# UZ-SLAMLab/ORB_SLAM3

Hardware: AMD Instinct MI355X
Metric: ORB kfeatures/sec extract+match, EuRoC 752x480 nFeatures=1000 (higher is better)
Workload: dtype u8

## Files before the change

include/orbx.h:

```cpp
#ifndef ORBX_H
#define ORBX_H

#include <stddef.h>
#include <stdint.h>

#ifdef __cplusplus
extern "C" {
#endif

#define ORBX_VERSION 100

enum {
    ORBX_OK = 0,
    ORBX_E_EMPTY = -1,
    ORBX_E_BAD_ARG = -2,
    ORBX_E_TOO_SMALL = -3,
    ORBX_E_CAPACITY = -4,
    ORBX_E_NO_DEVICE = -5,
    ORBX_E_HIP = -6,
    ORBX_E_TOO_LARGE = -7,
    ORBX_E_INTERNAL = -8,
    ORBX_E_STALE = -9
};

// ... 52 lines not shown
int orbx_batch_download(orbx_extractor *ex, int frame, orbx_keypoint *keypoints, uint8_t *descriptors, int cap,
                        int *n_out, int *mono_index);
int orbx_batch_download_all(orbx_extractor *ex, orbx_keypoint *keypoints, uint8_t *descriptors, int32_t *counts,
                            int32_t *mono_index);
int orbx_output_capacity(orbx_extractor *ex, int width, int height);
int orbx_batch_download_async(orbx_extractor *ex, orbx_keypoint *keypoints, uint8_t *descriptors, int32_t *counts,
                              int32_t *mono_index, int32_t *match, int32_t *nmatches);
int orbx_download_wait(orbx_extractor *ex);

int orbx_get_level(orbx_extractor *ex, int frame, int level, uint8_t *dst, size_t dst_stride);
int orbx_level_size(orbx_extractor *ex, int width, int height, int level, int *w, int *h);
int orbx_get_level_device(orbx_extractor *ex, int frame, int level, const uint8_t **d_padded, size_t *pitch);

int orbx_get_levels(const orbx_extractor *ex);
float orbx_get_scale_factor(const orbx_extractor *ex);
int orbx_get_scale_tables(const orbx_extractor *ex, float *scale, float *inv_scale, float *sigma2, float *inv_sigma2);
int orbx_get_feature_tables(const orbx_extractor *ex, int32_t *features_per_level, int32_t *umax16);

int orbx_debug_level_candidates(orbx_extractor *ex, int frame, int level, orbx_keypoint *out, int cap);
int orbx_debug_level_keypoints(orbx_extractor *ex, int frame, int level, orbx_keypoint *out, int cap);
int orbx_debug_level_blurred(orbx_extractor *ex, int frame, int level, uint8_t *dst, size_t dst_stride);
int orbx_debug_fused_patches(orbx_extractor *ex, int frame, uint8_t *dst, int cap_keypoints);
int orbx_debug_stage_stats(orbx_extractor *ex, int64_t *out, int cap);

int orbx_tune_fast_queues(orbx_extractor *ex, int mode, int32_t info[4]);

int orbx_profile_enable(orbx_extractor *ex, int enable);
int orbx_profile_read(orbx_extractor *ex, const char **names, double *avg_ms, int64_t *launches, int cap);

typedef struct orbx_matcher orbx_matcher;
int orbx_matcher_create(int device, orbx_matcher **out);
void orbx_matcher_destroy(orbx_matcher *m);
int orbx_matcher_debug_transfers(const orbx_matcher *m, int64_t *out, int cap);
int orbx_matcher_debug_replay_stats(const orbx_matcher *m, int32_t *out3);

#define ORBX_TH_LOW 50
#define ORBX_TH_HIGH 100
#define ORBX_HISTO_LENGTH 30

int orbx_hamming_csr(orbx_matcher *m, const uint8_t *q_desc, int n_q, const uint8_t *t_desc, int n_t,
                     const int32_t *row_ptr, const int32_t *cand, uint16_t *dist_out);

int orbx_hamming_best2_csr(orbx_matcher *m, const uint8_t *q_desc, int n_q, const uint8_t *t_desc, int n_t,
                           const int32_t *row_ptr, const int32_t *cand, int32_t *best_pos, int32_t *best_dist,
                           int32_t *second_pos, int32_t *second_dist);

// ... 271 lines not shown
```

orb_slam3_amd/_lib.py:

```python
from __future__ import annotations

import ctypes as C
import os
from pathlib import Path

import numpy as np

_PKG = Path(__file__).resolve().parent
LIB_PATH = _PKG / "liborbx.so"

KP_DTYPE = np.dtype([("x", "<f4"), ("y", "<f4"), ("size", "<f4"), ("angle", "<f4"), ("response", "<f4"),
                     ("octave", "<i4"), ("class_id", "<i4")])

ORBX_OK = 0
ORBX_E_EMPTY = -1
ORBX_E_STALE = -9
FLAG_DESC_STRICT = 1
FLAG_BLUR_OCV440 = 2
FLAG_ATAN_FMA = 4
TH_LOW, TH_HIGH, HISTO_LENGTH = 50, 100, 30


class OrbxError(RuntimeError):
    def __init__(self, status: int, where: str):
# ... 73 lines not shown
class BowKeyFrame(C.Structure):
    _fields_ = [("descriptors", C.c_void_p), ("angle", C.c_void_p), ("valid", C.c_void_p), ("n", C.c_int32), ("fv", FeatVec)]


MAX_BOW_KEYFRAMES = 1024


class FuseQueries(C.Structure):
    _fields_ = [("n", C.c_int32), ("u", C.c_void_p), ("v", C.c_void_p), ("ur", C.c_void_p), ("r", C.c_void_p), ("level", C.c_void_p),
                ("desc", C.c_void_p)]


MAX_FUSE_KEYFRAMES = 256

PAIR_PREDICATE = C.CFUNCTYPE(C.c_int, C.c_void_p, C.c_int, C.c_int)

_lib = None

SYMBOLS = [
    "orbx_create", "orbx_destroy", "orbx_extract", "orbx_extract_batch_device", "orbx_extract_batch_host", "orbx_batch_view_get", "orbx_sync",
    "orbx_batch_download", "orbx_batch_download_all", "orbx_batch_download_async", "orbx_download_wait", "orbx_output_capacity", "orbx_get_level", "orbx_level_size",
    "orbx_get_level_device", "orbx_get_levels", "orbx_get_scale_factor", "orbx_get_scale_tables",
    "orbx_get_feature_tables", "orbx_debug_level_candidates", "orbx_debug_level_keypoints",
    "orbx_debug_level_blurred", "orbx_debug_stage_stats", "orbx_tune_fast_queues", "orbx_debug_fused_patches", "orbx_profile_enable", "orbx_profile_read", "orbx_matcher_create",
    "orbx_matcher_destroy", "orbx_matcher_debug_transfers", "orbx_matcher_debug_replay_stats", "orbx_hamming_csr", "orbx_hamming_best2_csr", "orbx_knn2", "orbx_stereo_rowband",
    "orbx_compute_stereo_matches", "orbx_search_by_projection_mappoints", "orbx_search_by_projection_frame",
    "orbx_match_consecutive_device", "orbx_last_error", "orbx_status_string", "orbx_search_by_projection_window", "orbx_search_by_projection_mappoints_fisheye", "orbx_search_by_projection_frame_fisheye",
    "orbx_search_by_bow_frame_fisheye", "orbx_undistort_keypoints", "orbx_image_bounds", "orbx_is_in_frustum", "orbx_is_in_frustum_checks", "orbx_frustum_batch_device",
    "orbx_set_camera", "orbx_batch_download_keypoints_un",
    "orbx_search_for_initialization", "orbx_search_by_bow_frame", "orbx_search_by_bow_keyframes",
    "orbx_search_for_triangulation", "orbx_search_for_triangulation_pinhole", "orbx_search_for_triangulation_kb8", "orbx_debug_kb8_epipolar", "orbx_stereo_batch_device", "orbx_stereo_batch_download", "orbx_stereo_batch_download_all", "orbx_stereo_batch_download_async", "orbx_stereo_download_wait", "orbx_search_mappoints_batch_device", "orbx_vocabulary_create",
    "orbx_vocabulary_destroy", "orbx_bow_transform", "orbx_distinctive_descriptors", "orbx_fuse_search",
    "orbx_frame_create", "orbx_frame_destroy", "orbx_frame_load_host", "orbx_frame_load_batch", "orbx_frame_count",
    "orbx_frame_search_by_projection_mappoints", "orbx_frame_search_by_projection_frame", "orbx_frame_search_local_points",
    "orbx_compute_stereo_fisheye_matches", "orbx_stereo_fisheye_batch_device", "orbx_stereo_fisheye_batch_download",
    "orbx_stereo_fisheye_batch_download_all",
    "orbx_vocabulary_set_word_weights", "orbx_frame_compute_bow", "orbx_frame_search_by_bow", "orbx_frame_search_by_projection_window",
    "orbx_frame_load_host_fisheye", "orbx_frame_load_stereo_fisheye_batch", "orbx_frame_counts", "orbx_frame_search_by_projection_mappoints_fisheye",
    "orbx_frame_search_by_projection_frame_fisheye", "orbx_frame_search_local_points_fisheye",
    "orbx_frame_compute_bow_fisheye", "orbx_frame_search_by_bow_fisheye", "orbx_frame_search_by_projection_window_fisheye",
    "orbx_keyframe_from_frame", "orbx_keyframe_create_host", "orbx_keyframe_count", "orbx_keyframe_destroy", "orbx_keyframe_fuse_search",
    "orbx_keyframe_fuse_map_points",
]


def lib() -> C.CDLL:
    global _lib
# ... 12 lines not shown
    L.orbx_destroy.argtypes = [vp]
    L.orbx_extract.argtypes = [vp, vp, i32, i32, sz, i32, i32, vp, vp, i32, vp, vp]
    L.orbx_extract_batch_device.argtypes = [vp, vp, i32, i32, i32, sz, sz, i32, i32]
    L.orbx_extract_batch_host.argtypes = [vp, vp, i32, i32, i32, sz, sz, i32, i32]
    L.orbx_batch_view_get.argtypes = [vp, C.POINTER(BatchView)]
    L.orbx_sync.argtypes = [vp]
    L.orbx_batch_download.argtypes = [vp, i32, vp, vp, i32, vp, vp]
    L.orbx_batch_download_all.argtypes = [vp, vp, vp, vp, vp]
    L.orbx_output_capacity.argtypes = [vp, i32, i32]
    L.orbx_batch_download_async.argtypes = [vp, vp, vp, vp, vp, vp, vp]
    L.orbx_download_wait.argtypes = [vp]
    L.orbx_get_level.argtypes = [vp, i32, i32, vp, sz]
    L.orbx_level_size.argtypes = [vp, i32, i32, i32, vp, vp]
    L.orbx_get_level_device.argtypes = [vp, i32, i32, vp, vp]
    L.orbx_get_levels.argtypes = [vp]
    L.orbx_get_scale_factor.argtypes = [vp]
    L.orbx_get_scale_factor.restype = f32
    L.orbx_get_scale_tables.argtypes = [vp, vp, vp, vp, vp]
    L.orbx_get_feature_tables.argtypes = [vp, vp, vp]
    L.orbx_debug_level_candidates.argtypes = [vp, i32, i32, vp, i32]
    L.orbx_debug_level_keypoints.argtypes = [vp, i32, i32, vp, i32]
    L.orbx_debug_level_blurred.argtypes = [vp, i32, i32, vp, sz]
    L.orbx_debug_stage_stats.argtypes = [vp, vp, i32]
    L.orbx_tune_fast_queues.argtypes = [vp, i32, vp]
    L.orbx_debug_fused_patches.argtypes = [vp, i32, vp, i32]
    L.orbx_debug_sort_nodes.argtypes = [i32, vp, vp, i32, vp]
    L.orbx_debug_sort_nodes_par.argtypes = [i32, vp, vp, i32, vp, vp]
    L.orbx_profile_enable.argtypes = [vp, i32]
    L.orbx_profile_read.argtypes = [vp, vp, vp, vp, i32]
    L.orbx_matcher_create.argtypes = [i32, C.POINTER(vp)]
    L.orbx_matcher_destroy.argtypes = [vp]
    L.orbx_matcher_debug_transfers.argtypes = [vp, vp, i32]
    L.orbx_matcher_debug_replay_stats.argtypes = [vp, vp]
    L.orbx_hamming_csr.argtypes = [vp, vp, i32, vp, i32, vp, vp, vp]
    L.orbx_hamming_best2_csr.argtypes = [vp, vp, i32, vp, i32, vp, vp, vp, vp, vp, vp]
    L.orbx_knn2.argtypes = [vp, vp, i32, vp, i32, vp, vp]
    L.orbx_stereo_rowband.argtypes = [vp, vp, vp, i32, vp, vp, i32, vp, i32, i32, f32, f32, vp, vp]
    L.orbx_compute_stereo_matches.argtypes = [vp, vp, vp, i32, vp, vp, i32, vp, vp, i32, vp, vp, vp, vp, vp, f32, f32,
                                              vp, vp]
    L.orbx_search_by_projection_mappoints.argtypes = [vp, C.POINTER(FrameDesc), vp, i32, vp, vp, vp, vp, vp, vp, vp,
                                                      vp, f32, f32, vp]
    L.orbx_search_by_projection_frame.argtypes = [vp, C.POINTER(FrameDesc), vp, i32, vp, vp, vp, vp, vp, vp, vp, f32,
                                                  i32, i32, vp]
    L.orbx_search_by_projection_mappoints_fisheye.argtypes = [vp, C.POINTER(FrameDesc), vp, i32, vp, vp, vp, i32] + [vp] * 12 + [f32, f32, vp]
    L.orbx_search_by_projection_frame_fisheye.argtypes = [vp, C.POINTER(FrameDesc), vp, i32, vp, i32] + [vp] * 8 + [f32, i32, i32, vp]
    L.orbx_search_by_bow_frame_fisheye.argtypes = [vp, vp, vp, vp, i32, C.POINTER(FeatVec), vp, vp, i32, i32, C.POINTER(FeatVec), f32, i32, vp]
# ... 79 lines not shown
```

orb_slam3_amd/csrc/extractor_state.h:

```cpp
#pragma once

#include <hip/hip_runtime.h>

#include <cstdio>
#include <cstdlib>
#include <string>
#include <vector>

#include "orbx_internal.h"

namespace orbx {

extern thread_local std::string g_last_error;
void set_error(const std::string &s);

#define ORBX_HIP(expr)                                                                                 \
    do {                                                                                               \
        hipError_t _e = (expr);                                                                        \
        if (_e != hipSuccess) {                                                                        \
            orbx::set_error(std::string(#expr) + ": " + hipGetErrorString(_e));                        \
            return ORBX_E_HIP;                                                                         \
        }                                                                                              \
    } while (0)

// ... 66 lines not shown
    typedef orbx::DevBuf DevBuf;
    typedef orbx::LevelInfo LevelInfo;
    enum { K_COUNT = orbx::K_COUNT };
    orbx_params prm;
    int device = 0;
    hipStream_t stream = nullptr;
    std::vector<float> scale, inv_scale, sigma2, inv_sigma2;
    std::vector<int> quota;
    int umax[16];
    int width = 0, height = 0, batch_cap = 0, last_batch = 0;
    std::vector<LevelInfo> lv;
    size_t pyr_frame = 0, blur_frame = 0, cand_frame = 0, lvl_frame = 0;
    int total_cells = 0, cap = 0, max_pool = 0;
    size_t fast_lds = 0;
    bool resize_march_ok[orbx::kMaxLevels] = {};
    bool fast_strip = false;
    static constexpr int kStripGcap0 = 512, kStripQcap0 = 816;
    int strip_gmax = 1024, strip_qmax = 4096;
    int n_strips = 0, strip_pix_bytes = 0, strip_gcap = kStripGcap0, strip_qcap = kStripQcap0;
    int fast_wave_pitch = 64, fast_wave_rows = 0, fast_wave_qfull = 16;
    DevBuf d_fast_ovf;
    bool oct_par = true;
    bool oct_single_wave = false;
    bool fast_wave = true;
    int n_fast_tiles = 0, n_blur_items = 0;
    int blur_waves = 2048;
    DevBuf d_lv, d_xtab, d_ytab, d_xgtab, d_fast_tiles, d_strips, d_blur_items, d_dc;
    struct PyrPlanDev { DevBuf cols, steps, tasks, band0; orbx::PyrStreamGeom geom; int bands = 0; size_t lds = 0; bool ok = false; };
    PyrPlanDev ps_plan[4];
    bool ps_ok = false;
    int ps_wg_target = 512;
    int ps_min_frames = 48;
    bool lvl0_inplace = false;
    bool in0_released = false;
    unsigned in0_copy_seq = 0;
    hipEvent_t in0_event = nullptr;
    const uint8_t *in0_images = nullptr;
    size_t in0_row_stride = 0, in0_frame_stride = 0;
    int n_strips0 = 0;
    DevBuf d_pyr2;
    bool pyr_double = false;
    int pyr_slot = 0;
    uint8_t *pyr_cur() const { return (uint8_t *)(pyr_slot ? d_pyr2.p : d_pyr.p); }
    DevBuf d_pyr, d_blur, d_cellcnt, d_cellent, d_keys0, d_keys1, d_nof0, d_nof1, d_lvlkp, d_lvlcnt, d_candtot, d_work;
    DevBuf d_kps, d_desc, d_count, d_mono, d_err;
    DevBuf d_mkey1, d_mkey2, d_mocc, d_mentries, d_mprobs, d_mres, d_mscale, d_mgrid;
// ... 70 lines not shown
```

orb_slam3_amd/csrc/octree_par.hip.h:

```cpp
#pragma once

#include "octree.hip.h"

namespace orbx {

constexpr int kOctParLdsKeys = 4096;
constexpr int kOctTier1Keys = 1792;
constexpr int kOctBlkE = 17;

#define OCT_WAVE_SYNC() do { __builtin_amdgcn_fence(__ATOMIC_SEQ_CST, "workgroup"); __builtin_amdgcn_wave_barrier(); } while (0)

__host__ __device__ inline size_t oct_par_pool_bytes(int pool) {
    return ((size_t)kOctStackInts * 4 + (size_t)pool * (16 + 16 + 16 + 8 + 16 + 14) + 160 + 15) & ~(size_t)15;
}
__host__ __device__ inline size_t oct_par_lds_bytes(int pool) { return oct_par_pool_bytes(pool) + (size_t)kOctParLdsKeys * 6; }

struct OctBnd { int16_t x0, y0, x1, y1; };
struct OctSeg { int32_t beg, cnt; };

__device__ __forceinline__ uint64_t oct_readlane64(uint64_t v, int l) {
    return ((uint64_t)(uint32_t)__builtin_amdgcn_readlane((int)(v >> 32), l) << 32) | (uint32_t)__builtin_amdgcn_readlane((int)v, l);
}
__device__ __forceinline__ int oct_median3(uint64_t va, uint64_t vb, uint64_t vc, int ia, int ib, int ic) {
    if (oct_less(va, vb)) {
        if (oct_less(vb, vc)) return ib;
        if (oct_less(va, vc)) return ic;
        return ia;
    }
    if (oct_less(va, vc)) return ia;
    if (oct_less(vb, vc)) return ic;
// ... 160 lines not shown
    const int tid = threadIdx.x, lane = tid & 63, w = tid >> 6;
    int run = 0;
    for (int c0 = 0; c0 < ncell; c0 += 256) {
        const int c = c0 + tid;
        const int n = (c < ncell) ? ccnt[c] : 0;
        const int incl = wave_incl_scan(n);
        if (lane == 63) wsum[w] = incl;
        __syncthreads();
        const int s0 = wsum[0], s1 = wsum[1], s2 = wsum[2], s3 = wsum[3];
        __syncthreads();
        const int excl = run + incl - n + (w > 0 ? s0 : 0) + (w > 1 ? s1 : 0) + (w > 2 ? s2 : 0);
        const uint32_t *src = ent + (size_t)c * L.cell_cap;
        for (int k = 0; k < n; k += 4) {
            uint32_t v[4];
#pragma unroll
            for (int u = 0; u < 4; u++) v[u] = (k + u < n) ? src[k + u] : 0u;
#pragma unroll
            for (int u = 0; u < 4; u++) if (k + u < n) dst[excl + k + u] = v[u];
        }
        run += s0 + s1 + s2 + s3;
    }
    return run;
}
template <int CTRL, int ROWS>
__device__ __forceinline__ void oct_seg_step(uint32_t &lo, uint32_t &hi, int &f) {
    const uint32_t plo = (uint32_t)__builtin_amdgcn_update_dpp(0, (int)lo, CTRL, ROWS, 0xf, false);
    const uint32_t phi = (uint32_t)__builtin_amdgcn_update_dpp(0, (int)hi, CTRL, ROWS, 0xf, false);
    const int pf = __builtin_amdgcn_update_dpp(0, f, CTRL, ROWS, 0xf, false);
    if (!f) { lo += plo; hi += phi; }
    f |= pf;
}
__device__ __forceinline__ uint64_t oct_blk_seg_excl(uint64_t v, bool fl, uint64_t *wtot, int *wflag, int lane, int wave) {
    uint32_t lo = (uint32_t)v, hi = (uint32_t)(v >> 32);
    int f = fl ? 1 : 0;
    oct_seg_step<0x111, 0xf>(lo, hi, f);
    oct_seg_step<0x112, 0xf>(lo, hi, f);
    oct_seg_step<0x114, 0xf>(lo, hi, f);
    oct_seg_step<0x118, 0xf>(lo, hi, f);
    oct_seg_step<0x142, 0xa>(lo, hi, f);
    oct_seg_step<0x143, 0xc>(lo, hi, f);
    if (lane == 63) { wtot[wave] = ((uint64_t)hi << 32) | lo; wflag[wave] = f; }
    __syncthreads();
    const uint32_t elo = (uint32_t)__builtin_amdgcn_update_dpp(0, (int)lo, 0x138, 0xf, 0xf, false);
    const uint32_t ehi = (uint32_t)__builtin_amdgcn_update_dpp(0, (int)hi, 0x138, 0xf, 0xf, false);
    const int ef = __builtin_amdgcn_update_dpp(0, f, 0x138, 0xf, 0xf, false);
    const uint64_t ev = ((uint64_t)ehi << 32) | elo;
// ... 525 lines not shown
    OCT_SYNC_ALL();
    for (int i = tid; i < C; i += NT) {
        const uint32_t key = kb[cur][i];
        atomicMax(&best[nof[cur][i]], ((uint32_t)key_s(key) << 20) | (0xfffffu - (uint32_t)i));
    }
    OCT_SYNC_ALL();
    for (int i = tid; i < nn && i < L.lvl_cap; i += NT) {
        const uint32_t key = kb[cur][0xfffffu - (best[i] & 0xfffffu)];
        out[i] = pack_key(key_x(key) + kBorder, key_y(key) + kBorder, key_s(key));
    }
    if (tid == 0) {
        if (nn > L.lvl_cap) atomicExch(err, 3);
        *lvlcnt_out = min(nn, L.lvl_cap);
    }
    OCT_TICK(6);
    if (dbg && tid == 0) { dbg[0] += (long long)wall_clock64() - tstart; dbg[9] = C; dbg[11] = nn; }
#undef OCT_TICK
#undef OCT_SYNC_ALL
}

__device__ __forceinline__ bool oct_blk_form(const LevelInfo &L, int C) { return C <= kOctParLdsKeys && L.nIni <= 4 && L.pool <= 2047; }

template <int KEYS, int LO>
__global__ __launch_bounds__(256, (KEYS <= 2048 ? 5 : 3)) void k_octree_par_t(const LevelInfo *__restrict__ lv, size_t ent_frame_stride,
                                                                              uint32_t *__restrict__ keys1, uint32_t *__restrict__ lvlkp,
                                                                              size_t lvlkp_frame_stride, int32_t *__restrict__ lvlcnt, int nlevels,
                                                                              int32_t *__restrict__ cand_total, int32_t *__restrict__ err,
                                                                              int max_pool, const int32_t *__restrict__ cellcnt, int total_cells,
                                                                              const uint32_t *__restrict__ cellent) {
    extern __shared__ __attribute__((aligned(16))) uint8_t smem[];
    const int level = blockIdx.y, f = blockIdx.x;
    const LevelInfo L = lv[level];
    uint32_t *gk1 = keys1 + (size_t)f * ent_frame_stride + L.cand_off;
    int C;
    if (LO < 0 && cellcnt) {
        C = __builtin_amdgcn_readfirstlane(compact_level(L, cellcnt + (size_t)f * total_cells + L.cell_base,
                                                         cellent + (size_t)f * ent_frame_stride + L.cand_off, gk1));
        if (threadIdx.x == 0) cand_total[f * nlevels + level] = C;
        __syncthreads();
    } else C = __builtin_amdgcn_readfirstlane(cand_total[f * nlevels + level]);
    if (!(C > LO && C <= KEYS && L.nIni <= 4 && L.pool <= 2047)) return;
    octree_par_body<true, KEYS>(L, smem, max_pool, C, nullptr, gk1, nullptr, nullptr, lvlkp + (size_t)f * lvlkp_frame_stride + L.lvl_off,
                                lvlcnt + f * nlevels + level, err, nullptr);
}

__global__ __launch_bounds__(256, 3) void k_octree_rest(const LevelInfo *__restrict__ lv, size_t ent_frame_stride, uint32_t *__restrict__ keys0,
                                                        uint32_t *__restrict__ keys1, uint16_t *__restrict__ nof0, uint16_t *__restrict__ nof1,
                                                        uint32_t *__restrict__ lvlkp, size_t lvlkp_frame_stride, int32_t *__restrict__ lvlcnt,
                                                        int nlevels, const int32_t *__restrict__ cand_total, int32_t *__restrict__ err, int max_pool, int single_wave) {
    extern __shared__ __attribute__((aligned(16))) uint8_t smem[];
    const int level = blockIdx.y, f = blockIdx.x;
    const LevelInfo L = lv[level];
    int32_t *cnt_out = lvlcnt + f * nlevels + level;
    const int C = __builtin_amdgcn_readfirstlane(cand_total[f * nlevels + level]);
    uint32_t *gk1 = keys1 + (size_t)f * ent_frame_stride + L.cand_off;
    if (oct_blk_form(L, C)) {
        if (C <= kOctTier1Keys) return;
        octree_par_body<true, kOctParLdsKeys>(L, smem, max_pool, C, nullptr, gk1, nullptr, nullptr, lvlkp + (size_t)f * lvlkp_frame_stride + L.lvl_off, cnt_out,
                                              err, nullptr);
        return;
    }
    uint32_t *gk0 = keys0 + (size_t)f * ent_frame_stride + L.cand_off;
// ... 16 lines not shown
```

orb_slam3_amd/csrc/orbx_extractor.hip:

```cpp
#include <hip/hip_runtime.h>

#include <algorithm>
#include <cmath>
#include <cstdio>
#include <cstdlib>
#include <cstring>
#include <dlfcn.h>
#include <mutex>
#include <string>
#include <vector>

#include "extractor_kernels.hip.h"
#include "geometry_kernels.hip.h"
#include "extractor_state.h"

namespace orbx {

thread_local std::string g_last_error;

void set_error(const std::string &s) { g_last_error = s; }

namespace {
struct Roctx {
    int (*push)(const char *) = nullptr;
// ... 526 lines not shown
    ex->n_strips = (int)strips.size();
    ex->n_strips0 = 0;
    {
        int gmax = 64, qmax = 256;
        for (const StripTile &T : strips) {
            const int bh = (T.ih + 3) / 4, G = (T.iw + 3) >> 2;
            gmax = std::max(gmax, bh * G); qmax = std::max(qmax, bh * 4 * G);
        }
        ex->strip_gmax = (gmax + 7) & ~7; ex->strip_qmax = (qmax + 15) & ~15;
        ex->strip_gcap = std::min(ex->strip_gcap, std::max(ex->strip_gmax, orbx_extractor::kStripGcap0));
        ex->strip_qcap = std::min(ex->strip_qcap, std::max(ex->strip_qmax, orbx_extractor::kStripQcap0));
    }
    for (const StripTile &T : strips) if (T.src_off < lv[0].off + (size_t)lv[0].pitch * (lv[0].h + 2 * kEdge)) ex->n_strips0++;
    ex->fast_strip = fast_strip && ex->fast_wave && !strips.empty();
    if (ex->strip_qcap > 2 * ex->strip_gcap) ex->strip_gcap = (ex->strip_qcap / 2 + 7) & ~7;
    if (getenv("ORBX_DEBUG_ALLOC"))
        fprintf(stderr, "[orbx fast] %s: %d strips per frame, %zu cells, pixel tile %d B, LDS %zu B per workgroup\n", ex->fast_strip ? "k_fast_strip" : "per-cell kernels",
                ex->n_strips, fast_tiles.size(), ex->strip_pix_bytes, fast_strip_lds_bytes(4, ex->strip_pix_bytes, ex->strip_gcap, ex->strip_qcap));
    ex->fast_wave_pitch = (fast_wave_maxw + 7 <= 48) ? 48 : 64;
    ex->fast_wave_rows = fast_wave_rows;
    ex->fast_wave_qfull = fast_wave_qfull;
    { const char *v = getenv("ORBX_OCTREE"); ex->oct_par = !(v && v[0] == 's') && oct_par_lds_bytes(max_pool) <= 150 * 1024;
      ex->oct_single_wave = v && v[0] == 'w'; }
    ex->n_fast_tiles = (int)fast_tiles.size(); ex->n_blur_items = (int)blur_items.size();
    ex->last_batch = 0;
    ex->batch_seq++;
    ex->lvl0_inplace = false;
    if (ex->has_camera) {
        CameraModel c = {ex->cam_params[0], ex->cam_params[1], ex->cam_params[2], ex->cam_params[3], ex->cam_params[4], ex->cam_params[5],
                         ex->cam_params[6], ex->cam_params[7], ex->cam_params[8]};
        image_bounds(c, width, height, ex->bounds);
    } else {
        ex->bounds[0] = 0.f; ex->bounds[1] = (float)width; ex->bounds[2] = 0.f; ex->bounds[3] = (float)height;
    }
    return ORBX_OK;
}

struct ProfScope {
    orbx_extractor *ex;
    int k;
    ProfScope(orbx_extractor *e, int kernel) : ex(e), k(kernel) {
        if (ex->profile) (void)hipEventRecord(ex->ev0, ex->stream);
    }
    ~ProfScope() {
        if (ex->profile) {
            (void)hipEventRecord(ex->ev1, ex->stream);
// ... 145 lines not shown
            ORBX_HIP(hipGetLastError());
            const size_t lds_full = fast_wave_lds_bytes(ex->fast_wave_pitch, ex->fast_wave_rows, ex->fast_wave_qfull);
#define ORBX_FAST_WAVE_LIST(PITCH)                                                                                                  \
    hipLaunchKernelGGL(k_fast_wave_list<PITCH>, dim3(n < 8 ? 256 : 4096), dim3(64), lds_full, st, d_lv, (const TileRef *)ex->d_fast_tiles.p,         \
                       (const uint8_t *)pyr, ex->pyr_frame, (int32_t *)ex->d_cellcnt.p, ex->total_cells, (uint32_t *)ex->d_cellent.p, \
                       ex->cand_frame, ini, mn, ex->fast_wave_rows, ex->fast_wave_qfull, (const uint32_t *)ovf_list,                  \
                       (const int32_t *)ovf_count, src0)
            if (ex->fast_wave_pitch == 48) ORBX_FAST_WAVE_LIST(48); else ORBX_FAST_WAVE_LIST(64);
#undef ORBX_FAST_WAVE_LIST
        } else {
            hipLaunchKernelGGL(k_fast_cells<64>, dim3(ex->n_fast_tiles, n), dim3(64), ex->fast_lds, st, d_lv, (const TileRef *)ex->d_fast_tiles.p,
                               (const uint8_t *)pyr, ex->pyr_frame, (int32_t *)ex->d_cellcnt.p, ex->total_cells, (uint32_t *)ex->d_cellent.p,
                               ex->cand_frame, ini, mn);
        }
    }
    {
        ProfScope ps(ex, K_OCTREE);
        if (ex->oct_par) {
            const size_t lds = oct_par_lds_bytes(ex->max_pool), lds1 = oct_par_pool_bytes(ex->max_pool);
            const size_t lds_s = oct_par_pool_bytes(ex->max_pool) + (size_t)kOctTier1Keys * 6;
            const size_t lds_r = std::max(lds, lds1);
            if (lds_r > 64 * 1024) ORBX_HIP(hipFuncSetAttribute((const void *)k_octree_rest, hipFuncAttributeMaxDynamicSharedMemorySize, (int)lds_r));
            if (lds_s > 64 * 1024) ORBX_HIP(hipFuncSetAttribute((const void *)k_octree_par_t<kOctTier1Keys, -1>, hipFuncAttributeMaxDynamicSharedMemorySize, (int)lds_s));
            hipLaunchKernelGGL((k_octree_par_t<kOctTier1Keys, -1>), dim3(n, nl), dim3(256), lds_s, st, d_lv, ex->cand_frame, (uint32_t *)ex->d_keys1.p,
                               (uint32_t *)ex->d_lvlkp.p, ex->lvl_frame, (int32_t *)ex->d_lvlcnt.p, nl, (int32_t *)ex->d_candtot.p,
                               (int32_t *)ex->d_err.p, ex->max_pool, (const int32_t *)ex->d_cellcnt.p,
                               ex->total_cells, (const uint32_t *)ex->d_cellent.p);
            hipLaunchKernelGGL(k_octree_rest, dim3(n, nl), dim3(256), lds_r, st, d_lv, ex->cand_frame, (uint32_t *)ex->d_keys0.p,
                               (uint32_t *)ex->d_keys1.p, (uint16_t *)ex->d_nof0.p, (uint16_t *)ex->d_nof1.p, (uint32_t *)ex->d_lvlkp.p,
                               ex->lvl_frame, (int32_t *)ex->d_lvlcnt.p, nl, (const int32_t *)ex->d_candtot.p, (int32_t *)ex->d_err.p,
                               ex->max_pool, ex->oct_single_wave ? 1 : 0);
        } else {
            if (oct_lds_bytes(ex->max_pool) > 64 * 1024)
                ORBX_HIP(hipFuncSetAttribute((const void *)k_octree, hipFuncAttributeMaxDynamicSharedMemorySize, (int)oct_lds_bytes(ex->max_pool)));
            hipLaunchKernelGGL(k_octree, dim3(nl, n), dim3(64), oct_lds_bytes(ex->max_pool), st, d_lv,
                               (const int32_t *)ex->d_cellcnt.p, ex->total_cells, (const uint32_t *)ex->d_cellent.p, ex->cand_frame,
                               (uint32_t *)ex->d_keys0.p, (uint32_t *)ex->d_keys1.p, (uint32_t *)ex->d_lvlkp.p, ex->lvl_frame,
                               (int32_t *)ex->d_lvlcnt.p, nl, (int32_t *)ex->d_candtot.p, (int32_t *)ex->d_err.p, ex->max_pool);
        }
    }
    if (ex->copy_pending) {
        ORBX_HIP(hipStreamWaitEvent(st, ex->ev_copy_done[(ex->copy_issued - 1) & 1], 0));
    }
    if (ex->match_pending && !(ex->copy_pending && ex->copy_covers_match)) {
        ORBX_HIP(hipStreamWaitEvent(st, ex->ev_match, 0));
    }
    {
        ProfScope ps(ex, K_FINALIZE);
        hipLaunchKernelGGL(k_finalize, dim3(n), dim3(256), 0, st, d_lv, nl, (const uint32_t *)ex->d_lvlkp.p, ex->lvl_frame,
                           (const int32_t *)ex->d_lvlcnt.p, (WorkItem *)ex->d_work.p, ex->cap, (int32_t *)ex->d_count.p,
                           (int32_t *)ex->d_mono.p, lap0, lap1, (int32_t *)ex->d_err.p);
    }
    if (!ex->fused_blur && !ex->profile && ex->side_streams) ORBX_HIP(hipStreamWaitEvent(st, ex->ev_blur, 0));
    {
// ... 111 lines not shown
        const int vmax = (int)std::floor(kHalfPatch * std::sqrt(2.f) / 2 + 1);
        const int vmin = (int)std::ceil(kHalfPatch * std::sqrt(2.f) / 2);
        const double hp2 = kHalfPatch * kHalfPatch;
        for (v = 0; v < 16; v++) ex->umax[v] = 0;
        for (v = 0; v <= vmax; ++v) ex->umax[v] = cv_round_d(std::sqrt(hp2 - v * v));
        for (v = kHalfPatch, v0 = 0; v >= vmin; --v) {
            while (ex->umax[v0] == ex->umax[v0 + 1]) ++v0;
            ex->umax[v] = v0;
            ++v0;
        }
    }
    const int prio_lo = 0, prio_hi = 0;
    hipError_t e = hipStreamCreateWithPriority(&ex->stream, hipStreamNonBlocking, prio_hi);
    if (e != hipSuccess) { set_error(hipGetErrorString(e)); delete ex; return ORBX_E_HIP; }
    (void)hipEventCreate(&ex->ev0);
    (void)hipEventCreate(&ex->ev1);
    (void)hipStreamCreateWithPriority(&ex->copy_stream, hipStreamNonBlocking, prio_lo);
    { const char *v = getenv("ORBX_FAST_QCAP"); if (v && atoi(v) >= 16) ex->strip_qcap = atoi(v) & ~15; }
    (void)hipStreamCreateWithPriority(&ex->aux_stream, hipStreamNonBlocking, prio_hi);
    (void)hipStreamCreateWithPriority(&ex->match_stream, hipStreamNonBlocking, prio_lo);
    (void)hipStreamCreateWithPriority(&ex->in_stream, hipStreamNonBlocking, prio_hi);
    (void)hipStreamCreateWithFlags(&ex->spare_stream, hipStreamNonBlocking);
    for (hipEvent_t *ev : {&ex->ev_in_free[0], &ex->ev_in_free[1], &ex->ev_in_ready[0], &ex->ev_in_ready[1]}) (void)hipEventCreateWithFlags(ev, hipEventDisableTiming);
    for (hipEvent_t *ev : {&ex->ev_pyr, &ex->ev_blur, &ex->ev_describe, &ex->ev_match}) (void)hipEventCreateWithFlags(ev, hipEventDisableTiming);
    (void)hipEventCreateWithFlags(&ex->ev_copy_done[0], hipEventDisableTiming);
    (void)hipEventCreateWithFlags(&ex->ev_copy_done[1], hipEventDisableTiming);
    (void)hipHostMalloc((void **)&ex->h_err, 2 * sizeof(int32_t), hipHostMallocDefault);
    if (ex->h_err) { ex->h_err[0] = 0; ex->h_err[1] = 0; }
    DescConst dc;
    memset(&dc, 0, sizeof(dc));
    int n = 0;
    for (int u = 0; u <= kHalfPatch; u++) {
        int vm = -1;
        for (int v = 0; v <= kHalfPatch; v++) if (ex->umax[v] >= u) vm = v;
        dc.vmax_of_u[u] = (int8_t)vm;
        if (vm >= 0) n += (u == 0 ? 1 : 2) * (2 * vm + 1);
    }
    for (int r = 0; r < 31; r++)
        for (int ax = 0; ax < 4; ax++)
            for (int t = 0; t < 40; t++) {
                const int v = r - kHalfPatch, u = t - 18 - ax;
                if (std::abs(u) <= ex->umax[std::abs(v)]) dc.ic_mask[r][ax][t >> 2] |= 0xffu << (8 * (t & 3));
            }
    bool mono = true;
    for (int v = 0; v < kHalfPatch; v++) mono = mono && ex->umax[v] >= ex->umax[v + 1];
    if (n != 749 || !mono) { set_error("orientation disc has " + std::to_string(n) + " pixels"); orbx_destroy(ex); return ORBX_E_INTERNAL; }
    memcpy(dc.pat, kPatternData, 1024);
    for (int i = 0; i < 1024; i++) dc.patf[i >> 2][i & 3] = (float)kPatternData[i];
    int r = ex->d_dc.ensure(sizeof(DescConst));
    if (r != ORBX_OK) { orbx_destroy(ex); return r; }
    if (hipMemcpy(ex->d_dc.p, &dc, sizeof(dc), hipMemcpyHostToDevice) != hipSuccess) { orbx_destroy(ex); return ORBX_E_HIP; }
    if (max_width > 0 && max_height > 0) {
        r = configure(ex, max_width, max_height, std::max(max_batch, 1));
        if (r != ORBX_OK) { orbx_destroy(ex); return r; }
    }
    *out = ex;
    return ORBX_OK;
}

void orbx_destroy(orbx_extractor *ex) {
    if (!ex) return;
    (void)hipSetDevice(ex->device);
    if (ex->stream) (void)hipStreamSynchronize(ex->stream);
    for (hipStream_t s : {ex->copy_stream, ex->aux_stream, ex->match_stream, ex->in_stream, ex->spare_stream})
        if (s) { (void)hipStreamSynchronize(s); (void)hipStreamDestroy(s); }
    for (hipEvent_t ev : {ex->ev_in_free[0], ex->ev_in_free[1], ex->ev_in_ready[0], ex->ev_in_ready[1]}) if (ev) (void)hipEventDestroy(ev);
    ex->d_in[0].release(); ex->d_in[1].release();
    for (hipEvent_t ev : {ex->ev_pyr, ex->ev_blur, ex->ev_describe, ex->ev_match}) if (ev) (void)hipEventDestroy(ev);
    if (ex->ev_sf) (void)hipEventDestroy(ex->ev_sf);
    for (hipEvent_t ev : ex->ev_stereo_copy) if (ev) (void)hipEventDestroy(ev);
    for (hipEvent_t ev : ex->ev_copy_done) if (ev) (void)hipEventDestroy(ev);
    if (ex->h_err) (void)hipHostFree(ex->h_err);
    for (int i = 0; i < 3; i++) { if (ex->h_frustum[i]) (void)hipHostFree(ex->h_frustum[i]); if (ex->ev_frustum[i]) (void)hipEventDestroy(ex->ev_frustum[i]); }
    ex->d_match.release(); ex->d_nmatch.release();
    for (DevBuf *b : {&ex->d_st_bidx, &ex->d_st_bdist, &ex->d_st_ur, &ex->d_st_depth, &ex->d_st_sad, &ex->d_st_nm, &ex->d_st_scales, &ex->d_st_rowptr, &ex->d_st_rowidx}) b->release();
    for (DevBuf *b : {&ex->d_sf_idx, &ex->d_sf_dist, &ex->d_sf_l2r, &ex->d_sf_r2l, &ex->d_sf_depth, &ex->d_sf_p3d, &ex->d_sf_cnt, &ex->d_sf_sigma, &ex->d_sf_rig}) b->release();
    DevBuf *bufs[] = {&ex->d_lv, &ex->d_xtab, &ex->d_ytab, &ex->d_fast_tiles, &ex->d_blur_items, &ex->d_dc, &ex->d_pyr, &ex->d_pyr2,
                      &ex->d_blur, &ex->d_cellcnt, &ex->d_cellent, &ex->d_keys0, &ex->d_keys1, &ex->d_nof0, &ex->d_nof1, &ex->d_fast_ovf, &ex->d_lvlkp, &ex->d_lvlcnt,
                      &ex->d_candtot, &ex->d_work, &ex->d_kps, &ex->d_desc, &ex->d_count, &ex->d_mono, &ex->d_err,
                      &ex->d_mkey1, &ex->d_mkey2, &ex->d_mocc, &ex->d_mentries, &ex->d_mprobs, &ex->d_mres, &ex->d_mscale, &ex->d_mgrid, &ex->d_xgtab,
                      &ex->d_mp_qr, &ex->d_mp_qmin, &ex->d_mp_qmax, &ex->d_mp_valid, &ex->d_mp_keys, &ex->d_mp_meta, &ex->d_mp_grid, &ex->d_mp_probs,
                      &ex->d_mp_res, &ex->d_mp_misc, &ex->d_mp_entries, &ex->d_kps_un, &ex->d_frustum_frames, &ex->d_strips,
                      &ex->ps_plan[0].cols, &ex->ps_plan[0].steps, &ex->ps_plan[0].tasks, &ex->ps_plan[0].band0, &ex->ps_plan[1].cols, &ex->ps_plan[1].steps,
                      &ex->ps_plan[1].tasks, &ex->ps_plan[1].band0, &ex->ps_plan[2].cols, &ex->ps_plan[2].steps, &ex->ps_plan[2].tasks, &ex->ps_plan[2].band0,
                      &ex->ps_plan[3].cols, &ex->ps_plan[3].steps, &ex->ps_plan[3].tasks, &ex->ps_plan[3].band0};
    for (DevBuf *b : bufs) b->release();
    if (ex->h_stage) (void)hipHostFree(ex->h_stage);
    if (ex->ev0) (void)hipEventDestroy(ex->ev0);
    if (ex->ev1) (void)hipEventDestroy(ex->ev1);
    if (ex->stream) (void)hipStreamDestroy(ex->stream);
    delete ex;
// ... 396 lines not shown
    if (!ex || !out || cap < 7 || ex->last_batch <= 0) return ORBX_E_BAD_ARG;
    ORBX_HIP(hipSetDevice(ex->device));
    ORBX_HIP(hipStreamSynchronize(ex->stream));
    const int nl = ex->prm.nlevels, B = ex->last_batch;
    const size_t cb = sizeof(int32_t) * (size_t)nl * B;
    int r = ex->d2h_staged_begin(64 + cb);
    if (r != ORBX_OK) return r;
    if ((r = ex->d2h_staged(0, ex->d_fast_ovf.p, 4)) != ORBX_OK) return r;
    if ((r = ex->d2h_staged(64, ex->d_candtot.p, cb)) != ORBX_OK) return r;
    ORBX_HIP(hipStreamSynchronize(ex->stream));
    int32_t listed = 0;
    memcpy(&listed, ex->staged(0), 4);
    const int32_t *ct = (const int32_t *)ex->staged(64);
    int64_t t1 = 0, t2 = 0, t3 = 0, total = 0, most = 0;
    for (int i = 0; i < nl * B; i++) {
        const int64_t c = ct[i];
        total += c; most = std::max(most, c);
        if (c <= kOctTier1Keys) t1++; else if (c <= kOctParLdsKeys) t2++; else t3++;
    }
    out[0] = ex->fast_strip ? listed : -1; out[1] = (int64_t)ex->total_cells * B; out[2] = t1; out[3] = t2; out[4] = t3; out[5] = total; out[6] = most;
    return 7;
}

int orbx_tune_fast_queues(orbx_extractor *ex, int mode, int32_t info[4]) {
    if (!ex || mode < 0 || mode > 2) return ORBX_E_BAD_ARG;
    ORBX_HIP(hipSetDevice(ex->device));
    int32_t listed = 0;
    const int64_t cells = (int64_t)ex->total_cells * std::max(ex->last_batch, 0);
    if (ex->last_batch > 0 && ex->fast_strip) {
        ORBX_HIP(hipStreamSynchronize(ex->stream));
        int r = ex->d2h_staged_begin(64);
        if (r != ORBX_OK) return r;
        if ((r = ex->d2h_staged(0, ex->d_fast_ovf.p, 4)) != ORBX_OK) return r;
        ORBX_HIP(hipStreamSynchronize(ex->stream));
        memcpy(&listed, ex->staged(0), 4);
    }
    const int g0 = ex->strip_gcap, q0 = ex->strip_qcap;
    const int gdef = orbx_extractor::kStripGcap0, qdef = orbx_extractor::kStripQcap0;
    if (mode == 2) { ex->strip_gcap = gdef; ex->strip_qcap = qdef; }
    else if (mode == 1 && ex->fast_strip && cells > 0) {
        const int gmax = std::max(ex->strip_gmax, gdef), qmax = std::max(ex->strip_qmax, qdef);
        if ((int64_t)listed * 10 > cells) {
            ex->strip_qcap = std::min(qmax, (2 * q0 + 15) & ~15);
            ex->strip_gcap = gmax;
        } else if ((int64_t)listed * 200 < cells && q0 > qdef) {
            ex->strip_qcap = std::max(qdef, (q0 / 2 + 15) & ~15);
// ... 72 lines not shown
```

orb_slam3_amd/extractor.py:

```python
from __future__ import annotations

import ctypes as C

import numpy as np

from . import _lib
from ._lib import KP_DTYPE, Params, check, ptr


class ORBextractor:
    HARRIS_SCORE = 0
    FAST_SCORE = 1

    def __init__(self, nfeatures: int, scaleFactor: float, nlevels: int, iniThFAST: int, minThFAST: int,
                 device: int = 0, flags: int = 0):
        self._L = _lib.lib()
        self._h = C.c_void_p()
        prm = Params(nfeatures, scaleFactor, nlevels, iniThFAST, minThFAST, flags)
        check(self._L.orbx_create(C.byref(prm), device, 0, 0, 0, C.byref(self._h)), "orbx_create")
        self.nfeatures, self.nlevels, self.device = nfeatures, nlevels, device
        self._last_shape = None
        self._cap_of = {}
        self._sf_shape = None

# ... 234 lines not shown
        return out[:n]

    def debug_blurred(self, level: int, frame: int = 0) -> np.ndarray:
        w, h = self.level_size(level)
        out = np.zeros((h, w), np.uint8)
        check(self._L.orbx_debug_level_blurred(self._h, frame, level, ptr(out), out.strides[0]), "blurred")
        return out

    def debug_fused_patches(self, frame: int = 0, cap: int = 4096) -> np.ndarray:
        out = np.zeros((cap, 37, 37), np.uint8)
        n = self._L.orbx_debug_fused_patches(self._h, frame, ptr(out), cap)
        if n < 0:
            raise RuntimeError(f"orbx_debug_fused_patches: {n}")
        return out[:n]

    def stage_stats(self) -> dict:
        out = (C.c_int64 * 8)()
        n = self._L.orbx_debug_stage_stats(self._h, out, 8)
        if n < 7:
            raise RuntimeError(f"orbx_debug_stage_stats: {n}")
        return {"fast_list_cells": int(out[0]), "cells": int(out[1]), "quadtrees_le_1792": int(out[2]), "quadtrees_le_4096": int(out[3]),
                "quadtrees_single_wave": int(out[4]), "fast_candidates": int(out[5]), "max_candidates_of_a_level": int(out[6])}

    def tune_fast_queues(self, mode: int = 1) -> dict:
        info = (C.c_int32 * 4)()
        r = self._L.orbx_tune_fast_queues(self._h, int(mode), info)
        if r < 0:
            raise RuntimeError(f"orbx_tune_fast_queues: {r}")
        return {"changed": bool(r), "fast_list_cells": int(info[0]), "cells": int(info[1]), "group_queue": int(info[2]), "pixel_queue": int(info[3])}

    def profile_enable(self, on=True):
        self._L.orbx_profile_enable(self._h, int(on))

    def profile_read(self):
        names = (C.c_char_p * 16)()
        ms = (C.c_double * 16)()
        cnt = (C.c_int64 * 16)()
        k = self._L.orbx_profile_read(self._h, names, ms, cnt, 16)
        return {names[i].decode(): (ms[i], cnt[i]) for i in range(k)}
```

Measured before the change: 329,400.

## Add small-level octree tier with higher occupancy on a forked side stream

```diff
diff --git a/include/orbx.h b/include/orbx.h
--- a/include/orbx.h
+++ b/include/orbx.h
@@ -98,6 +98,7 @@
 int orbx_debug_level_blurred(orbx_extractor *ex, int frame, int level, uint8_t *dst, size_t dst_stride);
 int orbx_debug_fused_patches(orbx_extractor *ex, int frame, uint8_t *dst, int cap_keypoints);
 int orbx_debug_stage_stats(orbx_extractor *ex, int64_t *out, int cap);
+int orbx_debug_octree_tiers(orbx_extractor *ex, int32_t *out, int cap);
 
 int orbx_tune_fast_queues(orbx_extractor *ex, int mode, int32_t info[4]);
 
diff --git a/orb_slam3_amd/_lib.py b/orb_slam3_amd/_lib.py
--- a/orb_slam3_amd/_lib.py
+++ b/orb_slam3_amd/_lib.py
@@ -119,7 +119,7 @@
     "orbx_batch_download", "orbx_batch_download_all", "orbx_batch_download_async", "orbx_download_wait", "orbx_output_capacity", "orbx_get_level", "orbx_level_size",
     "orbx_get_level_device", "orbx_get_levels", "orbx_get_scale_factor", "orbx_get_scale_tables",
     "orbx_get_feature_tables", "orbx_debug_level_candidates", "orbx_debug_level_keypoints",
-    "orbx_debug_level_blurred", "orbx_debug_stage_stats", "orbx_tune_fast_queues", "orbx_debug_fused_patches", "orbx_profile_enable", "orbx_profile_read", "orbx_matcher_create",
+    "orbx_debug_level_blurred", "orbx_debug_stage_stats", "orbx_debug_octree_tiers", "orbx_tune_fast_queues", "orbx_debug_fused_patches", "orbx_profile_enable", "orbx_profile_read", "orbx_matcher_create",
     "orbx_matcher_destroy", "orbx_matcher_debug_transfers", "orbx_matcher_debug_replay_stats", "orbx_hamming_csr", "orbx_hamming_best2_csr", "orbx_knn2", "orbx_stereo_rowband",
     "orbx_compute_stereo_matches", "orbx_search_by_projection_mappoints", "orbx_search_by_projection_frame",
     "orbx_match_consecutive_device", "orbx_last_error", "orbx_status_string", "orbx_search_by_projection_window", "orbx_search_by_projection_mappoints_fisheye", "orbx_search_by_projection_frame_fisheye",
@@ -178,6 +178,7 @@
     L.orbx_debug_level_keypoints.argtypes = [vp, i32, i32, vp, i32]
     L.orbx_debug_level_blurred.argtypes = [vp, i32, i32, vp, sz]
     L.orbx_debug_stage_stats.argtypes = [vp, vp, i32]
+    L.orbx_debug_octree_tiers.argtypes = [vp, vp, i32]
     L.orbx_tune_fast_queues.argtypes = [vp, i32, vp]
     L.orbx_debug_fused_patches.argtypes = [vp, i32, vp, i32]
     L.orbx_debug_sort_nodes.argtypes = [i32, vp, vp, i32, vp]
diff --git a/orb_slam3_amd/csrc/extractor_state.h b/orb_slam3_amd/csrc/extractor_state.h
--- a/orb_slam3_amd/csrc/extractor_state.h
+++ b/orb_slam3_amd/csrc/extractor_state.h
@@ -112,6 +112,10 @@
     DevBuf d_fast_ovf;
     bool oct_par = true;
     bool oct_single_wave = false;
+    int oct_t0_bound = 0, oct_t0_pool = 0;
+    uint32_t oct_t0_levels = 0;
+    bool oct_t0_beside = true;
+    hipEvent_t ev_oct_fork = nullptr, ev_oct_join = nullptr;
     bool fast_wave = true;
     int n_fast_tiles = 0, n_blur_items = 0;
     int blur_waves = 2048;
diff --git a/orb_slam3_amd/csrc/octree_par.hip.h b/orb_slam3_amd/csrc/octree_par.hip.h
--- a/orb_slam3_amd/csrc/octree_par.hip.h
+++ b/orb_slam3_amd/csrc/octree_par.hip.h
@@ -6,6 +6,8 @@
 
 constexpr int kOctParLdsKeys = 4096;
 constexpr int kOctTier1Keys = 1792;
+constexpr int kOctTier0Keys = 768;
+constexpr int kOctTier0Wgs = 8;
 constexpr int kOctBlkE = 17;
 
 #define OCT_WAVE_SYNC() do { __builtin_amdgcn_fence(__ATOMIC_SEQ_CST, "workgroup"); __builtin_amdgcn_wave_barrier(); } while (0)
@@ -212,6 +214,12 @@
     }
     return run;
 }
+__device__ __forceinline__ int level_key_count(const LevelInfo &L, const int32_t *__restrict__ ccnt) {
+    const int ncell = L.nCols * L.nRows, lane = threadIdx.x & 63;
+    int s = 0;
+    for (int c = lane; c < ncell; c += 64) s += ccnt[c];
+    return __builtin_amdgcn_readlane(wave_incl_scan(s), 63);
+}
 template <int CTRL, int ROWS>
 __device__ __forceinline__ void oct_seg_step(uint32_t &lo, uint32_t &hi, int &f) {
     const uint32_t plo = (uint32_t)__builtin_amdgcn_update_dpp(0, (int)lo, CTRL, ROWS, 0xf, false);
@@ -783,22 +791,26 @@
 __device__ __forceinline__ bool oct_blk_form(const LevelInfo &L, int C) { return C <= kOctParLdsKeys && L.nIni <= 4 && L.pool <= 2047; }
 
 template <int KEYS, int LO>
-__global__ __launch_bounds__(256, (KEYS <= 2048 ? 5 : 3)) void k_octree_par_t(const LevelInfo *__restrict__ lv, size_t ent_frame_stride,
-                                                                              uint32_t *__restrict__ keys1, uint32_t *__restrict__ lvlkp,
-                                                                              size_t lvlkp_frame_stride, int32_t *__restrict__ lvlcnt, int nlevels,
-                                                                              int32_t *__restrict__ cand_total, int32_t *__restrict__ err,
-                                                                              int max_pool, const int32_t *__restrict__ cellcnt, int total_cells,
-                                                                              const uint32_t *__restrict__ cellent) {
+__global__ __launch_bounds__(256, (KEYS <= kOctTier0Keys ? kOctTier0Wgs : KEYS <= 2048 ? 5 : 3)) void k_octree_par_t(
+    const LevelInfo *__restrict__ lv, size_t ent_frame_stride, uint32_t *__restrict__ keys1, uint32_t *__restrict__ lvlkp, size_t lvlkp_frame_stride,
+    int32_t *__restrict__ lvlcnt, int nlevels, int32_t *__restrict__ cand_total, int32_t *__restrict__ err, int max_pool,
+    const int32_t *__restrict__ cellcnt, int total_cells, const uint32_t *__restrict__ cellent, int tier0_bound, uint32_t tier0_levels) {
     extern __shared__ __attribute__((aligned(16))) uint8_t smem[];
+    constexpr bool kSmall = KEYS == kOctTier0Keys;
     const int level = blockIdx.y, f = blockIdx.x;
     const LevelInfo L = lv[level];
     uint32_t *gk1 = keys1 + (size_t)f * ent_frame_stride + L.cand_off;
     int C;
     if (LO < 0 && cellcnt) {
-        C = __builtin_amdgcn_readfirstlane(compact_level(L, cellcnt + (size_t)f * total_cells + L.cell_base,
-                                                         cellent + (size_t)f * ent_frame_stride + L.cand_off, gk1));
-        if (threadIdx.x == 0) cand_total[f * nlevels + level] = C;
-        __syncthreads();
+        const int32_t *ccnt = cellcnt + (size_t)f * total_cells + L.cell_base;
+        C = __builtin_amdgcn_readfirstlane(level_key_count(L, ccnt));
+        const bool small_owns = tier0_bound > 0 && ((tier0_levels >> level) & 1u) && C <= tier0_bound;
+        if (!kSmall && threadIdx.x == 0) cand_total[f * nlevels + level] = C;
+        if (kSmall != small_owns) C = -1;
+        else {
+            compact_level(L, ccnt, cellent + (size_t)f * ent_frame_stride + L.cand_off, gk1);
+            __syncthreads();
+        }
     } else C = __builtin_amdgcn_readfirstlane(cand_total[f * nlevels + level]);
     if (!(C > LO && C <= KEYS && L.nIni <= 4 && L.pool <= 2047)) return;
     octree_par_body<true, KEYS>(L, smem, max_pool, C, nullptr, gk1, nullptr, nullptr, lvlkp + (size_t)f * lvlkp_frame_stride + L.lvl_off,
diff --git a/orb_slam3_amd/csrc/orbx_extractor.hip b/orb_slam3_amd/csrc/orbx_extractor.hip
--- a/orb_slam3_amd/csrc/orbx_extractor.hip
+++ b/orb_slam3_amd/csrc/orbx_extractor.hip
@@ -572,6 +572,20 @@
     ex->fast_wave_qfull = fast_wave_qfull;
     { const char *v = getenv("ORBX_OCTREE"); ex->oct_par = !(v && v[0] == 's') && oct_par_lds_bytes(max_pool) <= 150 * 1024;
       ex->oct_single_wave = v && v[0] == 'w'; }
+    {
+        const char *v = getenv("ORBX_OCTREE_TIER0"), *b = getenv("ORBX_OCTREE_TIER0_BESIDE");
+        ex->oct_t0_bound = v ? std::min(std::max(atoi(v), 0), kOctTier0Keys) : kOctTier0Keys;
+        ex->oct_t0_beside = !(b && b[0] == '0');
+        ex->oct_t0_levels = 0; ex->oct_t0_pool = 0;
+        for (int l = 0; l < nl && l < 32; l++) {
+            const LevelInfo &L = lv[l];
+            if (L.nIni <= 4 && L.pool <= 2047 && (oct_par_pool_bytes(L.pool) + (size_t)kOctTier0Keys * 6) * kOctTier0Wgs <= 160 * 1024) {
+                ex->oct_t0_levels |= 1u << l;
+                ex->oct_t0_pool = std::max(ex->oct_t0_pool, L.pool);
+            }
+        }
+        if (!ex->oct_t0_levels) ex->oct_t0_bound = 0;
+    }
     ex->n_fast_tiles = (int)fast_tiles.size(); ex->n_blur_items = (int)blur_items.size();
     ex->last_batch = 0;
     ex->batch_seq++;
@@ -763,14 +777,28 @@
             const size_t lds_r = std::max(lds, lds1);
             if (lds_r > 64 * 1024) ORBX_HIP(hipFuncSetAttribute((const void *)k_octree_rest, hipFuncAttributeMaxDynamicSharedMemorySize, (int)lds_r));
             if (lds_s > 64 * 1024) ORBX_HIP(hipFuncSetAttribute((const void *)k_octree_par_t<kOctTier1Keys, -1>, hipFuncAttributeMaxDynamicSharedMemorySize, (int)lds_s));
+            const bool fork = ex->oct_t0_bound > 0 && ex->oct_t0_beside && !ex->profile && ex->side_streams;
+            if (ex->oct_t0_bound > 0) {
+                hipStream_t ts = fork ? ex->aux_stream : st;
+                if (fork) {
+                    ORBX_HIP(hipEventRecord(ex->ev_oct_fork, st));
+                    ORBX_HIP(hipStreamWaitEvent(ts, ex->ev_oct_fork, 0));
+                }
+                hipLaunchKernelGGL((k_octree_par_t<kOctTier0Keys, -1>), dim3(n, nl), dim3(256), oct_par_pool_bytes(ex->oct_t0_pool) + (size_t)kOctTier0Keys * 6, ts,
+                                   d_lv, ex->cand_frame, (uint32_t *)ex->d_keys1.p, (uint32_t *)ex->d_lvlkp.p, ex->lvl_frame, (int32_t *)ex->d_lvlcnt.p, nl,
+                                   (int32_t *)ex->d_candtot.p, (int32_t *)ex->d_err.p, ex->oct_t0_pool, (const int32_t *)ex->d_cellcnt.p, ex->total_cells,
+                                   (const uint32_t *)ex->d_cellent.p, ex->oct_t0_bound, ex->oct_t0_levels);
+                if (fork) ORBX_HIP(hipEventRecord(ex->ev_oct_join, ts));
+            }
             hipLaunchKernelGGL((k_octree_par_t<kOctTier1Keys, -1>), dim3(n, nl), dim3(256), lds_s, st, d_lv, ex->cand_frame, (uint32_t *)ex->d_keys1.p,
                                (uint32_t *)ex->d_lvlkp.p, ex->lvl_frame, (int32_t *)ex->d_lvlcnt.p, nl, (int32_t *)ex->d_candtot.p,
                                (int32_t *)ex->d_err.p, ex->max_pool, (const int32_t *)ex->d_cellcnt.p,
-                               ex->total_cells, (const uint32_t *)ex->d_cellent.p);
+                               ex->total_cells, (const uint32_t *)ex->d_cellent.p, ex->oct_t0_bound, ex->oct_t0_levels);
             hipLaunchKernelGGL(k_octree_rest, dim3(n, nl), dim3(256), lds_r, st, d_lv, ex->cand_frame, (uint32_t *)ex->d_keys0.p,
                                (uint32_t *)ex->d_keys1.p, (uint16_t *)ex->d_nof0.p, (uint16_t *)ex->d_nof1.p, (uint32_t *)ex->d_lvlkp.p,
                                ex->lvl_frame, (int32_t *)ex->d_lvlcnt.p, nl, (const int32_t *)ex->d_candtot.p, (int32_t *)ex->d_err.p,
                                ex->max_pool, ex->oct_single_wave ? 1 : 0);
+            if (fork) ORBX_HIP(hipStreamWaitEvent(st, ex->ev_oct_join, 0));
         } else {
             if (oct_lds_bytes(ex->max_pool) > 64 * 1024)
                 ORBX_HIP(hipFuncSetAttribute((const void *)k_octree, hipFuncAttributeMaxDynamicSharedMemorySize, (int)oct_lds_bytes(ex->max_pool)));
@@ -928,7 +956,7 @@
     (void)hipStreamCreateWithPriority(&ex->in_stream, hipStreamNonBlocking, prio_hi);
     (void)hipStreamCreateWithFlags(&ex->spare_stream, hipStreamNonBlocking);
     for (hipEvent_t *ev : {&ex->ev_in_free[0], &ex->ev_in_free[1], &ex->ev_in_ready[0], &ex->ev_in_ready[1]}) (void)hipEventCreateWithFlags(ev, hipEventDisableTiming);
-    for (hipEvent_t *ev : {&ex->ev_pyr, &ex->ev_blur, &ex->ev_describe, &ex->ev_match}) (void)hipEventCreateWithFlags(ev, hipEventDisableTiming);
+    for (hipEvent_t *ev : {&ex->ev_pyr, &ex->ev_blur, &ex->ev_describe, &ex->ev_match, &ex->ev_oct_fork, &ex->ev_oct_join}) (void)hipEventCreateWithFlags(ev, hipEventDisableTiming);
     (void)hipEventCreateWithFlags(&ex->ev_copy_done[0], hipEventDisableTiming);
     (void)hipEventCreateWithFlags(&ex->ev_copy_done[1], hipEventDisableTiming);
     (void)hipHostMalloc((void **)&ex->h_err, 2 * sizeof(int32_t), hipHostMallocDefault);
@@ -972,7 +1000,7 @@
         if (s) { (void)hipStreamSynchronize(s); (void)hipStreamDestroy(s); }
     for (hipEvent_t ev : {ex->ev_in_free[0], ex->ev_in_free[1], ex->ev_in_ready[0], ex->ev_in_ready[1]}) if (ev) (void)hipEventDestroy(ev);
     ex->d_in[0].release(); ex->d_in[1].release();
-    for (hipEvent_t ev : {ex->ev_pyr, ex->ev_blur, ex->ev_describe, ex->ev_match}) if (ev) (void)hipEventDestroy(ev);
+    for (hipEvent_t ev : {ex->ev_pyr, ex->ev_blur, ex->ev_describe, ex->ev_match, ex->ev_oct_fork, ex->ev_oct_join}) if (ev) (void)hipEventDestroy(ev);
     if (ex->ev_sf) (void)hipEventDestroy(ex->ev_sf);
     for (hipEvent_t ev : ex->ev_stereo_copy) if (ev) (void)hipEventDestroy(ev);
     for (hipEvent_t ev : ex->ev_copy_done) if (ev) (void)hipEventDestroy(ev);
@@ -1415,6 +1443,22 @@
     return 7;
 }
 
+int orbx_debug_octree_tiers(orbx_extractor *ex, int32_t *out, int cap) {
+    if (!ex || !out || ex->last_batch <= 0) return ORBX_E_BAD_ARG;
+    const int nl = ex->prm.nlevels, B = ex->last_batch;
+    if (cap < 3 + nl * B) return ORBX_E_BAD_ARG;
+    ORBX_HIP(hipSetDevice(ex->device));
+    ORBX_HIP(hipStreamSynchronize(ex->stream));
+    const size_t cb = sizeof(int32_t) * (size_t)nl * B;
+    int r = ex->d2h_staged_begin(cb);
+    if (r != ORBX_OK) return r;
+    if ((r = ex->d2h_staged(0, ex->d_candtot.p, cb)) != ORBX_OK) return r;
+    ORBX_HIP(hipStreamSynchronize(ex->stream));
+    out[0] = ex->oct_par ? ex->oct_t0_bound : 0; out[1] = (int32_t)ex->oct_t0_levels; out[2] = ex->oct_t0_pool;
+    memcpy(out + 3, ex->staged(0), cb);
+    return 3 + nl * B;
+}
+
 int orbx_tune_fast_queues(orbx_extractor *ex, int mode, int32_t info[4]) {
     if (!ex || mode < 0 || mode > 2) return ORBX_E_BAD_ARG;
     ORBX_HIP(hipSetDevice(ex->device));
diff --git a/orb_slam3_amd/extractor.py b/orb_slam3_amd/extractor.py
--- a/orb_slam3_amd/extractor.py
+++ b/orb_slam3_amd/extractor.py
@@ -280,6 +280,17 @@
         return {"fast_list_cells": int(out[0]), "cells": int(out[1]), "quadtrees_le_1792": int(out[2]), "quadtrees_le_4096": int(out[3]),
                 "quadtrees_single_wave": int(out[4]), "fast_candidates": int(out[5]), "max_candidates_of_a_level": int(out[6])}
 
+    def octree_tiers(self, batch: int = 1) -> dict:
+        n = 3 + self.nlevels * batch
+        out = np.zeros(n, np.int32)
+        r = self._L.orbx_debug_octree_tiers(self._h, ptr(out), n)
+        if r != n:
+            raise RuntimeError(f"orbx_debug_octree_tiers: {r}")
+        cand = out[3:].reshape(batch, self.nlevels).copy()
+        eligible = np.array([(int(out[1]) >> l) & 1 for l in range(self.nlevels)], bool)
+        return {"bound": int(out[0]), "eligible": eligible, "pool": int(out[2]), "candidates": cand,
+                "small": eligible[None, :] & (cand <= int(out[0])) & (int(out[0]) > 0)}
+
     def tune_fast_queues(self, mode: int = 1) -> dict:
         info = (C.c_int32 * 4)()
         r = self._L.orbx_tune_fast_queues(self._h, int(mode), info)
```

Measured after the change: 326,100. 1.0% lower.
